# xulinfei1996/koordinator

Hardware: AMD Instinct MI355X
Metric: pods scheduled/sec + node-evals/sec (% HBM roofline) at 5k and 100k nodes (higher is better)
Workload: dtype int64; 1 GPU; C2: 10000 pods x 5000 nodes, NodeResourcesFit(LeastAllocated cpu/mem/batch-cpu/batch-mem) + LoadAwareScheduling(defaults) + ElasticQuota(32 leaf quotas); nodes=5000, percentage_of_nodes_to_score=100, parallelism=single-gpu, batch_pods=64, candidates=32

## Files before the change

koordinator_amd/csrc/koordgpu.hip:

```cpp
#include <hip/hip_runtime.h>

#include <algorithm>
#include <chrono>
#include <cmath>
#include <condition_variable>
#include <cstdio>
#include <cstdlib>
#include <cstring>
#include <mutex>
#include <string>
#include <unordered_map>
#include <unordered_set>
#include <vector>

#include <rccl/rccl.h>

#include "ks_pass.h"
#include "ks_mono.h"
#include "ks_plan.h"
#include "ks_fq.h"
#include "ks_debug.h"
#include "ks_topo.h"
#include "ks_preempt.h"
#include "ks_summary.h"
// ... 135 lines not shown
  r.h_mem = (double)r.mem * 100.0;
  r.gpu_core = s.gpu_core[i];
  r.gpu_mem = s.gpu_mem[i];
  r.gpu_ratio = s.gpu_ratio[i];
  if (r.gpu_core != 0 || r.gpu_mem != 0 || r.gpu_ratio != 0) r.flags |= kPodHasGpu | kPodGpuReq;
  r.rdma = s.rdma ? s.rdma[i] : 0;
  r.joint = s.joint ? s.joint[i] : 0u;
  r._pad0 = 0;
  if (r.rdma > 0) r.flags |= kPodHasGpu;
  if (dev_on && (r.flags & kPodHasGpu)) r.flags |= kPodDevNoNom;
  if ((r.flags & kPodHasGpu) || s.stat_dyn[i]) r.flags |= kPodNormDyn;
  if (s.topo && (s.topo[i].flags & KS_TOPO_DYN)) r.flags |= kPodTopoDyn;
  r.cpu_bind = (r.flags & KS_POD_CPU_BIND) ? ((s.cpu_bind[i] & 0x1Fu) | ((uint32_t)(r.cpu / 1000) << 8)) : 0u;
  out[i] = r;
}


struct SelectArgs {
  const uint2* __restrict__ in;
  const int32_t* __restrict__ cursor;
  uint32_t* cand_chunk;
  uint2* cand_t;
  uint64_t* cand_bound;
  uint64_t* cand_top;
  uint64_t* cand_second;
  int32_t* cand_count;
  int32_t* cand_total;
  int64_t nchunks;
  int64_t c0, c1;
  int32_t total_pods, batch, k;
  int32_t* next_base;
  const int32_t* real_cursor;
  const PodRec* pods;
};


constexpr int kSelHistBins = 1024;
constexpr int kSelThreads = 256;
constexpr int kSelUnroll = 8;
constexpr size_t kSelScratch = 128;
constexpr int kSelBlocks = 2 * kMaxBatch;
__host__ __device__ inline size_t select_smem(int64_t nc) { return (size_t)nc * sizeof(uint2) + kSelHistBins * 4 + kSelScratch; }

__global__ __launch_bounds__(kSelThreads) void select_kernel(SelectArgs a) {
  extern __shared__ __attribute__((aligned(16))) uint2 srow[];
  const int tid = threadIdx.x;
  const int lane = tid & 63;
  const int wv = tid >> 6;
  const int32_t cursor = __builtin_amdgcn_readfirstlane(*a.cursor);
  if (a.next_base && blockIdx.x == 0 && tid == 0) {
    const int32_t rc = *a.real_cursor;
    *a.next_base = (cursor == rc && cursor < a.total_pods) ? cursor + min(a.batch, a.total_pods - cursor) : rc;
  }
  if (cursor < a.total_pods && (__builtin_amdgcn_readfirstlane(a.pods[cursor].flags) & kPodTopoDyn)) return;
  if (cursor >= a.total_pods) return;
  const int32_t np = min(a.batch, a.total_pods - cursor);
  static_assert(kMaxBatch == 64, "the XCD mapping below: 4 XCDs x 16 pods (and ks_fq.h's per-pod records)");
  const int32_t xcd = (int32_t)(blockIdx.x & 7u);
  if (xcd >= kMaxBatch / 16) return;
  const int32_t p = xcd * 16 + (int32_t)(blockIdx.x >> 3);
  if (p >= np) return;
  const int32_t K = a.k;
  const int64_t nc = a.c1 - a.c0;
  const uint2* in = a.in + (size_t)a.c0 * kMaxBatch + p;
  uint32_t* hist = reinterpret_cast<uint32_t*>(srow + nc);
  uint64_t* xw = reinterpret_cast<uint64_t*>(hist + kSelHistBins);
  int32_t cnt = 0;
  uint32_t hmax = 0;
  uint64_t top = 0;
  for (int i = tid; i < kSelHistBins; i += kSelThreads) hist[i] = 0u;
  for (int64_t e0 = tid; e0 < nc; e0 += (int64_t)kSelThreads * kSelUnroll) {
    uint2 v[kSelUnroll];
#pragma unroll
    for (int u = 0; u < kSelUnroll; ++u) {
      const int64_t e = e0 + (int64_t)u * kSelThreads;
      v[u] = e < nc ? in[(size_t)e * kMaxBatch] : make_uint2(0u, 0u);
    }
#pragma unroll
    for (int u = 0; u < kSelUnroll; ++u) {
      const int64_t e = e0 + (int64_t)u * kSelThreads;
      if (e < nc) {
        srow[e] = v[u];
        const uint32_t h = v[u].x >> 6;
        cnt += h != 0;
        hmax = h > hmax ? h : hmax;
        top = umax64(top, local_gkey(v[u].x, a.c0 + e));
      }
    }
  }
  cnt = wave_sum_i32(cnt);
  hmax = wave_max_u32(hmax);
  top = wave_max_u64(top);
  if (lane == 0) {
    xw[wv] = top;
    xw[4 + wv] = (uint64_t)(uint32_t)cnt | ((uint64_t)hmax << 32);
  }
  __syncthreads();
  cnt = 0;
  hmax = 0;
  top = 0;
#pragma unroll
  for (int w = 0; w < kSelThreads / 64; ++w) {
    top = umax64(top, xw[w]);
    cnt += (int32_t)(uint32_t)xw[4 + w];
    const uint32_t hm = (uint32_t)(xw[4 + w] >> 32);
    hmax = hm > hmax ? hm : hmax;
  }
  uint32_t t = 1;
  int32_t need_eq = 0x7fffffff;
  const bool exhaustive = cnt <= K;
  const bool use_hist = !exhaustive && hmax < kSelHistBins;
  if (use_hist) {
    for (int64_t e = tid; e < nc; e += kSelThreads) {
      const uint32_t h = srow[e].x >> 6;
      if (h) atomicAdd(&hist[h], 1u);
    }
    __syncthreads();
  }
  if (wv != 0) return;
  if (!exhaustive) {
    if (use_hist) {
      constexpr int B = kSelHistBins / 64;
      uint32_t mine[B];
      uint32_t part = 0;
#pragma unroll
      for (int i = 0; i < B; ++i) {
        mine[i] = hist[lane * B + i];
        part += mine[i];
      }
      uint32_t suf = part;
#pragma unroll
      for (int off = 1; off < 64; off <<= 1) {
        const uint32_t v = __shfl_down(suf, off, 64);
        suf += (lane + off < 64) ? v : 0u;
      }
      const uint32_t suf_next = suf - part;
      const bool here = suf >= (uint32_t)K && suf_next < (uint32_t)K;
      uint32_t tl = 0, gtl = 0;
      if (here) {
        uint32_t acc = suf_next;
        for (int i = B - 1; i >= 0; --i) {
          if (acc + mine[i] >= (uint32_t)K) {
            tl = (uint32_t)(lane * B + i);
            gtl = acc;
            break;
          }
          acc += mine[i];
        }
      }
      const uint64_t hb = __ballot(here);
// ... 21 lines not shown
  uint64_t bound = 0, second = 0;
  const int64_t etop = top ? gkey_node(top) / 64 - a.c0 : -1;
  const uint64_t lanemask_lt = (lane == 0) ? 0ull : ((~0ull) >> (64 - lane));
  for (int64_t e0 = 0; e0 < nc; e0 += 64) {
    const int64_t e = e0 + lane;
    const uint2 loc = e < nc ? srow[e] : make_uint2(0u, 0u);
    second = umax64(second, local_gkey(e == etop ? loc.y : loc.x, a.c0 + e));
    const uint32_t h = loc.x >> 6;
    const bool is_gt = h > t;
    const bool is_eq = (h == t) && h != 0;
    const uint64_t beq = __ballot(is_eq);
    const int32_t eq_rank = eq_taken + __popcll(beq & lanemask_lt);
    const bool take_eq = is_eq && eq_rank < need_eq;
    const bool take = is_gt || take_eq;
    const uint64_t btake = __ballot(take);
    if (take) {
      const int32_t pos = base + __popcll(btake & lanemask_lt);
      a.cand_chunk[p * K + pos] = (uint32_t)(a.c0 + e);
      a.cand_t[p * K + pos] = loc;
      if (take_eq && eq_rank == need_eq - 1) bound = local_gkey(loc.x, a.c0 + e);
    }
    base += __popcll(btake);
    eq_taken += __popcll(beq);
  }
  bound = wave_max_u64(bound);
  second = wave_max_u64(second);
  if (lane == 0) {
    a.cand_count[p] = base;
    a.cand_total[p] = cnt;
    a.cand_bound[p] = exhaustive ? 0ull : bound;
    a.cand_top[p] = top;
    a.cand_second[p] = second;
  }
}



struct MergeArgs {
  const unsigned char* __restrict__ gather;
  const int32_t* __restrict__ cursor;
  uint32_t* cand_chunk;
  uint2* cand_t;
  uint64_t* cand_bound;
  uint64_t* cand_top;
  uint64_t* cand_second;
  int32_t* cand_count;
  int32_t nslots, total_pods, batch, k;
};

__global__ __launch_bounds__(64) void merge_kernel(MergeArgs a) {
  const int lane = threadIdx.x;
  const int32_t cursor = __builtin_amdgcn_readfirstlane(*a.cursor);
  if (cursor >= a.total_pods) return;
  const int32_t np = min(a.batch, a.total_pods - cursor);
  const int32_t p = blockIdx.x;
  if (p >= np) return;
  const int32_t K = a.k;
  const CandSlot L = cand_slot_layout(K);
  int32_t total = 0;
  uint64_t top = 0;
  for (int32_t s = 0; s < a.nslots; ++s) {
    const unsigned char* b = a.gather + (size_t)s * L.bytes;
    total += reinterpret_cast<const int32_t*>(b + L.total)[p];
    top = umax64(top, reinterpret_cast<const uint64_t*>(b + L.top)[p]);
  }
  auto entry = [&](int32_t s, int32_t i, uint32_t& chunk, uint2& t) {
// ... 732 lines not shown
  DevPtr<> evbuf;
  size_t evbuf_bytes = 0;
  DevPtr<> sumbuf;
  size_t sumbuf_bytes = 0;
  HostPtr sumhost;
  size_t sumhost_bytes = 0;
  DevPtr<> ures;
  DevPtr<> dscratch;
  size_t dscratch_bytes = 0;
  DevPtr<int2> cpuset_list;
  int32_t* cpuset_n = nullptr;
  CpuSet* cpuset_out = nullptr;
  uint32_t* cpuset_split = nullptr;
  int64_t* numa_alloc = nullptr;
  int32_t cpuset_cap = 0;
  DevPtr<uint32_t> cand_chunk;
  DevPtr<uint2> cand_t;
  DevPtr<uint64_t> cand_bound;
  DevPtr<uint64_t> cand_top;
  DevPtr<uint64_t> cand_second;
  DevPtr<> pre_rsv;
  DevPtr<int32_t> cand_total;
  DevPtr<int32_t> cand_count;
  DevPtr<int32_t> cursor;
  DevPtr<unsigned long long> counters;
  DevPtr<unsigned long long> dev_M;
  DevPtr<unsigned long long> dcache;
  int64_t dcache_words = 0;
  int32_t batch = 64, k = 32;
  int32_t k_cfg = 32;
  CommitPlan plan;
  bool commit_fq = true;
  bool fq_keys = true;
  int32_t nranks = 1, rank = 0, vshards = 1;
  ncclComm_t comm = nullptr;
  struct LoopGroup* loop = nullptr;
  hipEvent_t lev[2][2] = {};
  int64_t loop_seq = 0;
  DevPtr<unsigned long long> loop_scratch;
  DevPtr<unsigned char> gather;
  size_t gather_bytes = 0;
  hipStream_t sstream = nullptr;
  hipStream_t cstream = nullptr;
  DevPtr<int32_t> pipe;
  DevPtr<unsigned long long> pipe_top;
  int64_t pipe_k = 0;
  int32_t pipe_mode = -1;
  std::vector<Snap> snaps() const {
    std::vector<Snap> v;
    auto add = [&v](bool loaded, const auto& regions) {
      if (loaded) v.insert(v.end(), std::begin(regions), std::end(regions));
    };
    add(quota.blob.get(), quota.snap);
    add(dev.blob.get(), dev.snap);
    add(cpus.loaded, cpus.snap);
    add(numa.blob.get(), numa.snap);
    add(rsv.blob.get(), rsv.snap);
    return v;
  }
  ks_stats stats{};
};

#define KS_FAIL(ctx, code, ...)                                        \
  do {                                                                 \
    char buf_[512];                                                    \
    snprintf(buf_, sizeof(buf_), __VA_ARGS__);                         \
// ... 205 lines not shown
      return KS_EINVAL;
    }
  }
  if (cfg->reservation.enable) {
    const int64_t fitla = 100 * ((cfg->fit.enable_score ? cfg->fit.plugin_weight : 0) +
                                 (cfg->loadaware.enable_score ? cfg->loadaware.plugin_weight : 0) +
                                 (cfg->numa.enable ? cfg->numa.plugin_weight : 0) +
                                 (cfg->deviceshare.enable ? cfg->deviceshare.plugin_weight : 0) +
                                 (cfg->balanced.enable ? cfg->balanced.plugin_weight : 0) +
                                 (cfg->taint.enable_score ? cfg->taint.plugin_weight : 0) +
                                 (cfg->affinity.enable_score ? cfg->affinity.plugin_weight : 0));
    if (cfg->reservation.plugin_weight <= fitla || cfg->reservation.plugin_weight > ((int64_t)1 << 40) ||
        (fitla + 1) * (kRsvOrderBase + 1) >= (1 << 26)) {
      g_create_error = "ks_create: Reservation plugin weight must exceed 100 x (Fit + LoadAware weights) (ks_rsv.h ranking)";
      return KS_EUNSUPPORTED;
    }
  }
  int ndev = 0;
  if (hipGetDeviceCount(&ndev) != hipSuccess || ndev == 0) {
    g_create_error = "ks_create: no HIP device available";
    return KS_EHIP;
  }
  if (cfg->device < 0 || cfg->device >= ndev) {
    g_create_error = "ks_create: device ordinal out of range";
    return KS_EINVAL;
  }
  ks_ctx* ctx = new ks_ctx();
  ctx->cfg = *cfg;
  ctx->device = cfg->device;
  ctx->batch = cfg->batch_pods > 0 ? std::min(cfg->batch_pods, kMaxBatch) : 64;
  ctx->k = ctx->k_cfg = cfg->candidates > 0 ? std::min(cfg->candidates, kMaxCand) : 32;
  ctx->commit_fq = env_i64("KS_COMMIT_FQ", 1, 0, 1) != 0;
  ctx->fq_keys = env_i64("KS_FQ_KEYS", 1, 0, 1) != 0;
  if (hipSetDevice(ctx->device) != hipSuccess || hipStreamCreateWithFlags(&ctx->stream.h, hipStreamNonBlocking) != hipSuccess) {
    g_create_error = "ks_create: cannot create HIP stream";
    delete ctx;
    return KS_EHIP;
  }
  const size_t cand_bytes = (size_t)2 * kMaxBatch * kMaxCand;
  if (dev_alloc(ctx, ctx->cand_chunk, cand_bytes * 4) != KS_OK || dev_alloc(ctx, ctx->cand_t, cand_bytes * 8) != KS_OK ||
      dev_alloc(ctx, ctx->cand_bound, 2 * kMaxBatch * 8) != KS_OK || dev_alloc(ctx, ctx->cand_top, 2 * kMaxBatch * 8) != KS_OK ||
      dev_alloc(ctx, ctx->cand_second, 2 * kMaxBatch * 8) != KS_OK ||
      dev_alloc(ctx, ctx->pre_rsv, (size_t)kMaxBatch * kPreRsvM * sizeof(PreRsvT<kNumaWide>)) != KS_OK ||
      dev_alloc(ctx, ctx->cand_total, 2 * kMaxBatch * 4) != KS_OK || dev_alloc(ctx, ctx->cand_count, 2 * kMaxBatch * 4) != KS_OK ||
      dev_alloc(ctx, ctx->cursor, 64) != KS_OK || dev_alloc(ctx, ctx->counters, 256) != KS_OK ||
      dev_alloc(ctx, ctx->dev_M, kNormRows * kMaxBatch * 8) != KS_OK) {
    g_create_error = ctx->err;
    ks_destroy(ctx);
    return KS_ENOMEM;
  }
  if (hipMemsetAsync(ctx->cand_count.get(), list_fill(), 2 * kMaxBatch * 4, ctx->stream) != hipSuccess ||
      hipMemsetAsync(ctx->cand_chunk.get(), list_fill(), cand_bytes * 4, ctx->stream) != hipSuccess ||
      hipMemsetAsync(ctx->cand_t.get(), list_fill(), cand_bytes * 8, ctx->stream) != hipSuccess ||
      hipStreamSynchronize(ctx->stream) != hipSuccess) {
    g_create_error = "ks_create: cannot clear the candidate lists";
    ks_destroy(ctx);
    return KS_EHIP;
  }
  *out = ctx;
  return KS_OK;
}

void ks_destroy(ks_ctx* ctx) {
  if (!ctx) return;
  if (ctx->stream) (void)hipStreamSynchronize(ctx->stream);
  for (int i = 0; i < kPipeEvents; ++i) {
// ... 1715 lines not shown
      for (int t = 0; t < KS_AFFINITY_TERMS; ++t) {
        r.req[t] = pc->affinity_required[t] ? pc->affinity_required[t][i] : 0;
        r.pref[t] = pc->affinity_preferred[t] ? pc->affinity_preferred[t][i] : 0;
        r.w[t] = pc->affinity_weight[t] ? pc->affinity_weight[t][i] : 0;
        dyn |= (ctx->kc.aff & 2) && r.w[t] != 0;
      }
      r.pwant = pc->host_ports ? pc->host_ports[i] : 0;
      r.pconf = pc->host_ports_conflict ? pc->host_ports_conflict[i] : 0;
      hd[(size_t)i] = dyn ? 1 : 0;
    }
    if (p > 0) {
      HIPCHK(ctx, hipMemcpyAsync(st.stat, hs.data(), (size_t)p * sizeof(PodStat), hipMemcpyHostToDevice, ctx->stream));
      HIPCHK(ctx, hipMemcpyAsync(s.stat_dyn, hd.data(), (size_t)p, hipMemcpyHostToDevice, ctx->stream));
    }
    if (p > 0) {
      HIPCHK(ctx, hipStreamSynchronize(ctx->stream));
    }
  } else {
    HIPCHK(ctx, hipMemsetAsync(s.stat_dyn, 0, (size_t)p, ctx->stream));
  }
  return KS_OK;
}

static int prep_stage(ks_ctx* ctx, PodStage& st, int32_t p) {
  if (p <= 0) return KS_OK;
  const int threads = 256;
  hipLaunchKernelGGL(prep_pods_kernel, dim3((p + threads - 1) / threads), dim3(threads), 0, ctx->stream, st.cols,
                     st.recs, p, ctx->cfg.loadaware.scaling_cpu, ctx->cfg.loadaware.scaling_memory,
                     (int32_t)(ctx->cfg.deviceshare.enable != 0));
  HIPCHK(ctx, hipGetLastError());
  return KS_OK;
}

static int validate_pods(ks_ctx* ctx, const ks_pod_cols* pc, int32_t p) {
  if (ctx->cfg.topology.enable) {
    if ((pc->topo_term_beg == nullptr) != (pc->topo_terms == nullptr) || (pc->topo_prop_beg == nullptr) != (pc->topo_props == nullptr))
      KS_FAIL(ctx, KS_EINVAL, "topology lists: an offset array without its list (or the reverse)");
    for (int32_t i = 0; pc->topo_term_beg && i < p; ++i) {
      const int32_t b = pc->topo_term_beg[i], e = pc->topo_term_beg[i + 1];
      if ((i == 0 && b != 0) || e < b || e - b > KS_TOPO_MAX_TERMS)
        KS_FAIL(ctx, KS_EINVAL, "pod %d: topology term offsets [%d, %d) (at most %d terms)", i, b, e, KS_TOPO_MAX_TERMS);
      for (int32_t t = b; t < e; ++t) {
        const uint64_t w = pc->topo_terms[t];
        const int kind = (int)(w & 0xF), key = (int)((w >> 8) & 0xFF), prop = (int)((w >> 16) & 0xFFFF);
        const int32_t param = (int32_t)(uint32_t)(w >> 32);
        if (kind < KS_TOPO_K_SPREAD_HARD || kind > KS_TOPO_K_SCORE || prop >= ctx->topo.nprops || key > ctx->topo.nkeys ||
            ((w >> 5) & 0x7) != 0 ||
            ((kind == KS_TOPO_K_SPREAD_HARD || kind == KS_TOPO_K_SPREAD_SOFT) && param < 1) ||
            (kind == KS_TOPO_K_SCORE && (param < -1000000 || param > 1000000)))
          KS_FAIL(ctx, KS_EINVAL, "pod %d: topology term %d (%#llx) malformed", i, t - b, (unsigned long long)w);
      }
    }
    for (int32_t i = 0; pc->topo_prop_beg && i < p; ++i) {
      const int32_t b = pc->topo_prop_beg[i], e = pc->topo_prop_beg[i + 1];
      if ((i == 0 && b != 0) || e < b) KS_FAIL(ctx, KS_EINVAL, "pod %d: topology property offsets [%d, %d)", i, b, e);
      for (int32_t k = b; k < e; ++k)
        if (pc->topo_props[k] < 0 || pc->topo_props[k] >= ctx->topo.nprops)
          KS_FAIL(ctx, KS_EINVAL, "pod %d: topology property %d outside [0, %d)", i, pc->topo_props[k], ctx->topo.nprops);
    }
  }
  for (int32_t i = 0; pc->flags && i < p; ++i)
    if (pc->flags[i] & KS_POD_UNMODELLED)
      KS_FAIL(ctx, KS_EUNSUPPORTED, "pod %d: requests the library does not model (FPGA, DeviceShare allocate hints, "
                                    "a reserve pod as the scheduling subject)", i);
  for (int32_t i = 0; pc->affinity_required_n && i < p; ++i)
    if (pc->affinity_required_n[i] < 0 || pc->affinity_required_n[i] > KS_AFFINITY_TERMS)
// ... 168 lines not shown
  ca.n = ctx->nodes.n;
  ca.nchunks = ctx->nodes.nchunks;
  ca.total_pods = total;
  ca.batch = batch;
  ca.k = ctx->k;
  ca.rowcols = ctx->rowcols.get();
  ca.rcap = plan.rcap;
  ca.rsv_bytes = (int32_t)plan.rsv_bytes;
  ca.dev_bytes = (int32_t)plan.dev_bytes;
  ca.stat_lds = plan.stat_lds ? 1 : 0;
  ca.dv = ctx->ddv.get();
  ca.dev_M = ctx->dev_M.get();
  ca.cpuset_list = ctx->cpuset_list.get();
  ca.cpuset_n = ctx->cpuset_n;
  ca.cpuset_split = ctx->cpuset_split;
  ca.numa_alloc = ctx->numa_alloc;
  ca.force = 0;
  ca.numa_bytes = (int32_t)plan.numa_bytes;
  ca.nv = ctx->dnv.get();
  ca.pipe_base = nullptr;
  ca.carry = nullptr;
  ca.pipe_follow = nullptr;
  ca.pipe_after = nullptr;
  ca.top_reset = nullptr;
  ca.pre_rsv = nullptr;
  ca.topo = ctx->cfg.topology.enable && st.topo.get() ? 1 : 0;
  ca.topo_const = (int32_t)(100 * ctx->cfg.topology.spread_weight);
  ca.topo_rec = st.topo.get();
  ca.topo_props = st.topo_props.get();
  ca.topo_count = ctx->topo.count;
  ca.topo_npad = ctx->nodes.npad;
  ca.topo_best = ctx->topo.scr ? &ctx->topo.scr->best_total : nullptr;
  ca.nomq = nullptr;
  return ca;
}

static FqLaunch fq_launcher(int nsc) { return nsc == 0 ? fq_launch_n0() : (nsc == 2 ? fq_launch_n2() : fq_launch_n4()); }

static int commit_attr_set(ks_ctx* ctx) {
  static const int64_t env_general = env_i64("KS_COMMIT_GENERAL", 0, 0, 2);
  static const int64_t env_pre = env_i64("KS_PRE_RSV", 1, 0, 1);
  CommitPlanIn in{};
  in.kc = ctx->kc;
  in.k_cfg = ctx->k_cfg;
  in.nchunks = ctx->nodes.nchunks;
  in.nsc = ctx->nodes.nsc;
  in.numa_w = ctx->numa.w;
  in.q = ctx->quota.q.q;
  in.dev_held_any = ctx->rsv.dev_held_any;
  in.commit_fq = ctx->commit_fq;
  in.fq_keys = ctx->fq_keys;
  in.general_mode = (int)env_general;
  in.pre_rsv = env_pre != 0;
  const CommitPlan& plan = ctx->plan = commit_plan(in);
  if (plan.status == PlanStatus::kHeldWide)
    KS_FAIL(ctx, KS_EUNSUPPORTED,
            "reservations holding devices together with a NUMA-policy node with more than %d NUMA nodes", kNumaDev);
  ctx->k = plan.k;
  if (plan.status == PlanStatus::kTooLarge)
    KS_FAIL(ctx, KS_EUNSUPPORTED, "too many nodes for the commit kernel's LDS (%lld nodes, %zu B)", (long long)ctx->nodes.n, plan.smem);
  hipError_t e = pass_launcher(plan.feat, ctx->nodes.nsc, plan.wide).commit_attr(plan.qcache, plan.smem);
  if (e != hipSuccess) KS_FAIL(ctx, KS_EHIP, "hipFuncSetAttribute(commit LDS %zu): %s", plan.smem, hipGetErrorString(e));
  if (plan.fq) {
    e = fq_launcher(ctx->nodes.nsc).commit_attr(plan.fq_keys, plan.fq_smem);
    if (e != hipSuccess) KS_FAIL(ctx, KS_EHIP, "hipFuncSetAttribute(fq commit LDS %zu): %s", plan.fq_smem, hipGetErrorString(e));
  }
// ... 508 lines not shown
    } else if (k > 0) {
      HIPCHK(ctx, hipStreamWaitEvent(fs, ctx->pev_com[(k - 1) % kPipeEvents], 0));
    }
    sa.fix = carry;
    sa.fix_cursor = ctx->cursor.get();
    sa.ppw = pipe->fix_ppw;
    rec(3, fs);
    if (patch) {
      sa.list_t = cset.t;
      sa.list_chunk = cset.chunk;
      sa.list_count = cset.count;
      sa.list_bound = cset.bound;
      sa.list_top = ctx->pipe_top.get() + (size_t)(k & 1) * kMaxBatch;
      sa.list_k = ctx->k;
      le = pl.sweep(pipe->list_blocks, fs, sa);
    } else {
      sweep(pipe->fix_blocks, fs);
    }
    HIPCHK(ctx, le);
    rec(3, fs);
    return KS_OK;
  };
  if (pipe && !patch)
    if (int rc = fix(); rc != KS_OK) return rc;
  SelectArgs se;
  se.in = sout;
  se.cursor = base;
  se.nchunks = ctx->nodes.nchunks;
  se.total_pods = ctx->staged.np;
  se.batch = ctx->batch;
  se.k = ctx->k;
  se.real_cursor = ctx->cursor.get();
  se.pods = ctx->st.recs;
  const CandSlot L = cand_slot_layout(ctx->k);
  rec(1, ss);
  for (int32_t v = 0; v < ctx->vshards; ++v) {
    const int32_t sh = ctx->rank * ctx->vshards + v;
    se.c0 = shard_lo(sh);
    se.c1 = shard_lo(sh + 1);
    se.next_base = (pipe && !patch && v == 0) ? ctx->pipe.get() + ((k + 1) & 1) : nullptr;
    if (S == 1) {
      se.cand_chunk = cset.chunk;
      se.cand_t = cset.t;
      se.cand_bound = cset.bound;
      se.cand_top = cset.top;
      se.cand_second = cset.second;
      se.cand_count = cset.count;
      se.cand_total = cset.total;
    } else {
      unsigned char* b = ctx->gather.get() + (size_t)sh * L.bytes;
      se.cand_chunk = (uint32_t*)(b + L.chunk);
      se.cand_t = (uint2*)(b + L.t);
      se.cand_bound = cset.bound;
      se.cand_top = (uint64_t*)(b + L.top);
      se.cand_second = cset.second;
      se.cand_count = (int32_t*)(b + L.count);
      se.cand_total = (int32_t*)(b + L.total);
    }
    hipLaunchKernelGGL(select_kernel, dim3(kSelBlocks), dim3(kSelThreads), select_smem(se.c1 - se.c0), ss, se);
  }
  if (S > 1) {
    if (ctx->comm || ctx->loop)
      if (int rc = exchange_allgather(ctx, (size_t)ctx->vshards * L.bytes, ss); rc != KS_OK) return rc;
    MergeArgs ma;
    ma.gather = ctx->gather.get();
    ma.cursor = base;
// ... 18 lines not shown
    HIPCHK(ctx, hipEventRecord(ctx->pev_sel[k % kPipeEvents], ss));
    HIPCHK(ctx, hipStreamWaitEvent(cs, ctx->pev_sel[k % kPipeEvents], 0));
  }
  const CommitPlan& plan = ctx->plan;
  CommitArgs ca = commit_args(ctx, ctx->st, ctx->staged.np, ctx->batch);
  if (pipe) {
    ca.pipe_base = base;
    ca.carry = carry;
  }
  ca.cand_chunk = cset.chunk;
  ca.cand_t = cset.t;
  ca.cand_bound = cset.bound;
  ca.cand_top = cset.top;
  ca.cand_second = cset.second;
  ca.cand_count = cset.count;
  if (patch) {
    ca.pipe_follow = ctx->pipe.get() + ((k + 1) & 1);
    ca.pipe_after = base;
    ca.cand_top = (const uint64_t*)(ctx->pipe_top.get() + (size_t)(k & 1) * kMaxBatch);
    ca.top_reset = ctx->pipe_top.get() + (size_t)(k & 1) * kMaxBatch;
  }
  if (!plan.mono && !pipe && pl.reserve_pre && plan.pre_reserve) ca.pre_rsv = ctx->pre_rsv.get();
  rec(2, cs);
  if (ca.pre_rsv) HIPCHK(ctx, pl.reserve_pre(ctx->batch, cs, ca));
  if (ctx->nom.q_on) {
    ca.nomq = ctx->nom.dq;
    HIPCHK(ctx, pl.commit_nom(plan.qcache, plan.smem, cs, ca));
    if (ctx->nom.q_owners > 0) {
      hipLaunchKernelGGL((nom_retire_kernel<>), dim3(1), dim3(64), 0, cs, ctx->nom.q, (const ks_result*)ctx->st.results,
                         (const int32_t*)ctx->cursor.get(), ctx->counters.get());
      HIPCHK(ctx, hipGetLastError());
    }
  } else if (plan.mono) HIPCHK(ctx, pl.commit_mono(plan.qcache, plan.mono_smem, cs, ca));
  else if (plan.fq && !patch) HIPCHK(ctx, fq_launcher(ctx->nodes.nsc).commit(plan.fq_keys, plan.fq_smem, cs, ca));
  else HIPCHK(ctx, pl.commit(plan.qcache, plan.smem, cs, ca));
  rec(2, cs);
  if (pipe) HIPCHK(ctx, hipEventRecord(ctx->pev_com[k % kPipeEvents], cs));
  ctx->pipe_k = k + 1;
  return cores_pass_refresh(ctx);
}

static int schedule_staged_impl(ks_ctx* ctx) {
  if (!ctx->nodes.blob.get()) KS_FAIL(ctx, KS_ESTATE, "schedule before ks_load_nodes");
  if (!ctx->nom.q_staged) KS_NOM_REFUSE(ctx, "ks_schedule_staged");
  if (ctx->staged.stale)
    KS_FAIL(ctx, KS_ESTATE, "ks_schedule_staged: the staged batch predates a table reload; call ks_stage_pods again");
  ctx->nom.q_on = false;
  if (ctx->nom.q_staged && !ctx->nom.h_rows.empty()) {
    if (ctx->nranks * ctx->vshards > 1 || ctx->comm || ctx->loop)
      KS_FAIL(ctx, KS_EUNSUPPORTED, "ks_schedule_staged: a nominated table is loaded (%zu pods) and the nodes are sharded "
                                    "(ks_shard_init): the queue with a table runs on one shard only",
              ctx->nom.h_rows.size());
    ctx->nom.q_on = true;
  }
  HIPCHK(ctx, hipSetDevice(ctx->device));
  bind_mode(ctx, ctx->staged.bind_required);
  ctx->staged.cpusets_clobbered = false;
  ctx->stats = ks_stats{};
  const int32_t np = ctx->staged.np;
  if (np == 0) return KS_OK;
  {
    if (int rc = commit_attr_set(ctx); rc != KS_OK) return rc;
    hipError_t e = hipSuccess;
    if (ctx->nom.q_on) {
      const PassLaunch npl = pass_launcher(ctx->plan.feat, ctx->nodes.nsc, ctx->plan.wide);
      if (!npl.commit_nom || ctx->cfg.topology.enable)
        KS_FAIL(ctx, KS_EUNSUPPORTED, "ks_schedule_staged: a nominated table with a plugin set it is not modelled with");
// ... 31 lines not shown
  if (ppw > ctx->batch) ppw = ctx->batch;
  const int64_t nwork = std::max<int64_t>(local_chunks, 1) * ((ctx->batch + ppw - 1) / ppw);
  const int sweep_blocks = (int)((std::max<int64_t>(1, std::min<int64_t>((nwork + 3) / 4, env_cap)) + 7) & ~7ll);
  if (ensure_cpuset_bufs(ctx, np) != KS_OK) return KS_ENOMEM;
  hipEvent_t t0 = take_event(ctx, 0), t1 = take_event(ctx, 1);
  if (ctx->cpuset_list.get()) {
    HIPCHK(ctx, hipMemsetAsync(ctx->cpuset_n, 0, 4, ctx->stream));
    HIPCHK(ctx, hipMemsetAsync(ctx->cpuset_out, 0, (size_t)np * sizeof(CpuSet), ctx->stream));
    HIPCHK(ctx, hipMemsetAsync(ctx->numa_alloc, 0, (size_t)np * 2 * ctx->numa.w * 8, ctx->stream));
  }
  HIPCHK(ctx, hipMemsetAsync(ctx->cursor.get(), 0, 4, ctx->stream));
  HIPCHK(ctx, hipMemsetAsync(ctx->counters.get(), 0, 256, ctx->stream));
  PipeShape pshape{};
  const PipeShape* pipe = nullptr;
  if (!ctx->nom.q_on && pipelined(ctx)) {
    if (ensure_pipe(ctx) != KS_OK) return KS_EHIP;
    static const int64_t env_patch = env_i64("KS_PIPE_PATCH", 1, 0, 1);
    pshape.patch = env_patch != 0 && ctx->kc.monotone;
    static const int64_t env_fix_ppw = env_i64("KS_PIPE_FIX_PPW", 0, 1, kMaxBatch);
    pshape.fix_ppw = (int32_t)std::min<int64_t>(env_fix_ppw > 0 ? env_fix_ppw : (pshape.patch ? 16 : 2), ctx->batch);
    const int64_t fwork = (int64_t)kMaxBatch * ((ctx->batch + pshape.fix_ppw - 1) / pshape.fix_ppw);
    pshape.fix_blocks = (int)((std::max<int64_t>(1, (fwork + 3) / 4) + 7) & ~7ll);
    pshape.list_blocks = (int)((((int64_t)ctx->batch * ctx->k + 3) / 4 + 7) & ~7ll);
    pipe = &pshape;
    HIPCHK(ctx, hipMemsetAsync(ctx->pipe.get(), 0, kPipeWords * 4, ctx->stream));
    if (pshape.patch) {
      HIPCHK(ctx, hipMemsetD32Async((hipDeviceptr_t)(ctx->pipe.get() + 1), std::min(ctx->batch, np), 1, ctx->stream));
      HIPCHK(ctx, hipMemsetAsync(ctx->pipe_top.get(), 0, 2 * kMaxBatch * 8, ctx->stream));
    }
    ctx->pipe_k = 0;
  }
  HIPCHK(ctx, hipEventRecord(t0, ctx->stream));
  if (prep_stage(ctx, ctx->st, np) != KS_OK) return KS_EHIP;
  hipStream_t cs = pipe ? ctx->cstream : ctx->stream;
  if (pipe) {
    HIPCHK(ctx, hipEventRecord(ctx->pev_com[kPipeEvents - 1], ctx->stream));
    HIPCHK(ctx, hipStreamWaitEvent(ctx->sstream, ctx->pev_com[kPipeEvents - 1], 0));
    if (cs != ctx->stream) HIPCHK(ctx, hipStreamWaitEvent(cs, ctx->pev_com[kPipeEvents - 1], 0));
  }
  std::vector<std::pair<int, size_t>> evs;
  size_t evn = 2;
  int32_t host_cursor = 0;
  int rounds = 0;
  auto one_pass = [&](std::vector<std::pair<int, size_t>>* ev) -> int {
    switch (ctx->nodes.nsc) {
      case 0: return launch_pass<0>(ctx, ppw, sweep_blocks, pipe, ev, &evn);
      case 2: return launch_pass<2>(ctx, ppw, sweep_blocks, pipe, ev, &evn);
      default: return launch_pass<4>(ctx, ppw, sweep_blocks, pipe, ev, &evn);
    }
  };
  hipGraphExec_t gexec = nullptr;
  static const int64_t env_graph = env_i64("KS_TOPO_GRAPH", 1, 0, 1);
  constexpr int32_t kGraphIters = 4;
  if (ctx->cfg.topology.enable && ctx->st.ndyn > 0 && !pipe && !ctx->cfg.profile && env_graph && !ctx->comm && !ctx->loop) {
    EvBuf eb;
    if (ev_buffers(ctx, eb) != KS_OK) return KS_ENOMEM;
    hipGraph_t graph = nullptr;
    HIPCHK(ctx, hipStreamBeginCapture(ctx->stream, hipStreamCaptureModeThreadLocal));
    int rc = KS_OK;
    for (int32_t i = 0; i < kGraphIters && rc == KS_OK; ++i) rc = one_pass(nullptr);
    const hipError_t ee = hipStreamEndCapture(ctx->stream, &graph);
    if (rc != KS_OK) {
      if (graph) (void)hipGraphDestroy(graph);
      return rc;
    }
    HIPCHK(ctx, ee);
// ... 1236 lines not shown
```

koordinator_amd/csrc/ks_fq.h:

```cpp
#pragma once

#include "ks_pass.h"

namespace ks {

struct __attribute__((aligned(16))) FqPod {
  uint32_t qmeta;
  uint32_t flags;
  uint32_t qword;
  int32_t second;
  uint64_t bound, top;
};
static_assert(sizeof(FqPod) == 32, "FqPod layout");
static_assert(kMaxBatch == 64 && kMaxCand <= 64 && kQuotaLdsRows < 0xFFFF && KS_QUOTA_DIMS <= 8, "FqPod packing");

template <int NSC>
__device__ __forceinline__ uint64_t fq_rescan(const DevNodes* dnp, const Cfg& cfg, const PodRec& pod, int64_t chunk,
                                              uint64_t touched_mask, int64_t n) {
  const int lane = threadIdx.x & 63;
  const int64_t node = chunk * 64 + lane;
  asm volatile("" : "+s"(dnp));
  const DevNodes d = *dnp;
  NodeReg<NSC> r;
  load_node<NSC>(cfg, d, node, node < n, r);
  const EvalOut o = eval_pod_node<NSC, false>(cfg, pod, r);
  const bool skip = o.reasons || ((touched_mask >> lane) & 1ull);
  return wave_max_u64(skip ? 0ull : gkey(o.total, node));
}

template <int NSC, bool KEYS>
__global__ __launch_bounds__(commit_threads(0)) void commit_fq_kernel(CommitArgs a) {
  constexpr int NT = commit_threads(0);
  extern __shared__ __attribute__((aligned(16))) unsigned char smem_raw[];
  const int32_t K = a.k;
  const CommitLayout lay = commit_layout(K, a.nchunks, true, (size_t)a.rsv_bytes, (size_t)a.dev_bytes, (size_t)a.numa_bytes,
                                         a.q.q, true, false, KEYS);
  SlotRow* rows = reinterpret_cast<SlotRow*>(smem_raw + lay.rows);
  PodRec* spods = reinterpret_cast<PodRec*>(smem_raw + lay.pods);
  ks_result* sres = reinterpret_cast<ks_result*>(smem_raw + lay.res);
  int64_t* raw = reinterpret_cast<int64_t*>(smem_raw + lay.raw);
  int64_t* rawtop = reinterpret_cast<int64_t*>(smem_raw + lay.rawtop);
  int64_t* rawrun = reinterpret_cast<int64_t*>(smem_raw + lay.rawrun);
  int64_t* pqreq = reinterpret_cast<int64_t*>(smem_raw + lay.pqreq);
  uint2* cand_t = reinterpret_cast<uint2*>(smem_raw + lay.cand_t);
  uint32_t* cand_chunk = reinterpret_cast<uint32_t*>(smem_raw + lay.cand_chunk);
  FqPod* precs = reinterpret_cast<FqPod*>(smem_raw + lay.snuma);
  QuotaRowsLds qview = quota_lds(smem_raw + lay.quota, a.q.q);
  QuotaRowsLds* qlds = &qview;
  unsigned long long* touched = reinterpret_cast<unsigned long long*>(smem_raw + lay.touched);
  int2* hdesc = reinterpret_cast<int2*>(smem_raw + lay.help);
  int32_t* hpend = reinterpret_cast<int32_t*>(smem_raw + lay.help + (size_t)kMaxBatch * 8);
  int32_t* hdone = hpend + 1;
  int32_t* heval = hpend + 2;
  uint32_t* skey = reinterpret_cast<uint32_t*>(smem_raw + lay.skey);
  unsigned long long* hready = reinterpret_cast<unsigned long long*>(smem_raw + lay.help + (size_t)kMaxBatch * 8 + 16);
  const int tid = threadIdx.x;
  const int lane = tid & 63;
  const int32_t cursor0 = __builtin_amdgcn_readfirstlane(*a.cursor);
  if (cursor0 >= a.total_pods) {
    if (threadIdx.x == 0) pipe_next(a, cursor0);
    return;
  }
  if (pipe_bubble(a, cursor0)) return;
  const int32_t np = topo_pass_pods(a, cursor0, min(a.batch, a.total_pods - cursor0));
  if (np == 0) return;
#ifdef KS_COMMIT_STAMPS
  uint64_t ph[8] = {0, 0, 0, 0, 0, 0, 0, 0};
  uint64_t tlast = __builtin_amdgcn_s_memtime();
#define KS_FSTAMP(i)                                   \
  do {                                                 \
    const uint64_t t_ = __builtin_amdgcn_s_memtime(); \
    ph[i] += t_ - tlast;                               \
    tlast = t_;                                        \
  } while (0)
#else
#define KS_FSTAMP(i) \
  do {               \
  } while (0)
#endif

  lds_copy<NT>(cand_chunk, a.cand_chunk, np * K, tid);
  lds_copy<NT>(cand_t, a.cand_t, np * K, tid);
  for (int32_t i = tid; i < np * KS_QUOTA_DIMS; i += NT) {
    const int32_t p = i / KS_QUOTA_DIMS, dd = i - p * KS_QUOTA_DIMS;
    pqreq[i] = a.pq.req[dd][cursor0 + p];
  }
  {
    const int64_t* src = reinterpret_cast<const int64_t*>(a.pods + cursor0);
    int64_t* dst = reinterpret_cast<int64_t*>(spods);
    const int32_t words = np * (int32_t)(sizeof(PodRec) / 8);
    lds_copy<NT>(dst, src, words, tid);
  }
  for (int64_t c = tid; c < a.nchunks; c += NT) touched[c] = 0ull;
  lds_rawtop<NT>(rawtop, a.cand_top, a.rowcols, np, tid);
  lds_rawtop<NT>(rawrun, a.cand_second, a.rowcols, np, tid);
  for (int32_t r = tid; r < a.q.q; r += NT) {
    qlds->parent[r] = a.q.parent[r];
    qlds->limit_mask[r] = a.q.limit_mask[r];
    qlds->min_mask[r] = a.q.min_mask[r];
  }
  for (int32_t i = tid; i < a.q.q * KS_QUOTA_DIMS; i += NT) {
    qlds->limit[i] = a.q.limit[i];
    qlds->used[i] = a.q.used[i];
    qlds->min[i] = a.q.min[i];
    qlds->npused[i] = a.q.npused[i];
  }
  if (tid < 64 && lane < np) {
    const int32_t cnt = a.cand_count[lane];
    const uint64_t second = a.cand_second[lane];
    const uint32_t pmask = a.pq.mask[cursor0 + lane];
    const int32_t quota = a.pods[cursor0 + lane].quota;
    FqPod r;
    r.bound = a.cand_bound[lane];
    r.top = a.cand_top[lane];
    r.flags = a.pods[cursor0 + lane].flags;
    r.qmeta = 0xFFFFu;
    if (quota >= 0) {
      const int32_t pp = a.q.parent[quota];
      r.qmeta = (uint32_t)(pp < 0 ? 0xFFFF : pp) | ((a.q.limit_mask[quota] & 0xFFu) << 16) |
                ((a.q.min_mask[quota] & 0xFFu) << 24);
    }
    r.qword = (uint32_t)(quota < 0 ? 0xFFFF : quota) | ((pmask & 0xFFu) << 16) | ((uint32_t)max(0, min(cnt, 64)) << 24);
    r.second = (int32_t)gkey_node(second);
    precs[lane] = r;
  }
  const void* my_col = nullptr;
  int32_t my_w = 8;
  if (tid < RF_N) {
    my_col = a.rowcols[lane].p;
    my_w = a.rowcols[lane].width;
  }
  if (tid == 0) {
    *hpend = 0;
    *hdone = 0;
    heval[0] = 0;
    heval[1] = 0;
    *hready = 0ull;
  }
  __syncthreads();
  if (tid >= (KEYS ? 192 : 128)) return;
  KS_FSTAMP(0);
  Cfg cfg{};
  {
    auto pin = [](int32_t v) {
      asm volatile("" : "+s"(v));
      return v;
    };
    cfg.fit_filter = pin(a.c.fit_filter);
    cfg.fit_score = pin(a.c.fit_score);
    cfg.fw_cpu = pin(a.c.fw_cpu);
    cfg.fw_mem = pin(a.c.fw_mem);
    cfg.fw_eph = pin(a.c.fw_eph);
#pragma unroll
    for (int k = 0; k < NSC; ++k) cfg.fw_sc[k] = pin(a.c.fw_sc[k]);
    cfg.fit_pw = pin(a.c.fit_pw);
    cfg.la_filter = pin(a.c.la_filter);
    cfg.la_score = pin(a.c.la_score);
    cfg.la_prod_usage = pin(a.c.la_prod_usage);
    cfg.lw_cpu = pin(a.c.lw_cpu);
    cfg.lw_mem = pin(a.c.lw_mem);
    cfg.la_pw = pin(a.c.la_pw);
    cfg.quota_enable = 1;
    cfg.quota_parent = pin(a.c.quota_parent);
// ... 307 lines not shown
  if (lane < nslots) {
    const DevNodes d = *a.dn;
    const SlotRow& r = rows[lane];
    const int64_t node = snode;
    gst(d.req_cpu + node, r.t[ST_FREE_CPU].c - r.t[ST_FREE_CPU].h);
    gst(d.req_mem + node, r.t[ST_FREE_MEM].c - r.t[ST_FREE_MEM].h);
    gst(d.req_eph + node, r.t[ST_FREE_EPH].c - r.t[ST_FREE_EPH].h);
    gst(d.nz_cpu + node, term_requested(r.t[ST_CPU]));
    gst(d.nz_mem + node, term_requested(r.t[ST_MEM]));
#pragma unroll
    for (int k = 0; k < KS_MAX_SCALARS; ++k) gst(d.req_sc[k] + node, r.t[ST_FREE_SC + k].c - r.t[ST_FREE_SC + k].h);
    gst(d.pod_count + node, r.pod_count);
    gst(d.la_term_cpu + node, term_requested(r.t[ST_LCPU]));
    gst(d.la_term_mem + node, term_requested(r.t[ST_LMEM]));
    gst(d.la_pterm_cpu + node, term_requested(r.t[ST_PLCPU]));
    gst(d.la_pterm_mem + node, term_requested(r.t[ST_PLMEM]));
  }
  for (int32_t i = lane; i < a.q.q * KS_QUOTA_DIMS; i += 64) {
    a.q.used[i] = qlds->used[i];
    a.q.npused[i] = qlds->npused[i];
  }
  pipe_carry(a, nslots, snode);
  if (a.top_reset) a.top_reset[lane] = 0ull;
  if (lane == 0) {
    *a.cursor = cursor0 + processed;
    pipe_next(a, cursor0 + processed);
    atomicAdd(&a.counters[0], 1ull);
    if (processed < np) atomicAdd(&a.counters[1], 1ull);
    atomicAdd(&a.counters[2], (unsigned long long)rescans);
    atomicAdd(&a.counters[3], (unsigned long long)misses);
    atomicAdd(&a.counters[15], (unsigned long long)fast);
#ifdef KS_COMMIT_STAMPS
    for (int i = 0; i < 7; ++i) atomicAdd(&a.counters[8 + i], (unsigned long long)ph[i]);
#endif
  }
#undef KS_FSTAMP
}

struct FqLaunch {
  hipError_t (*commit)(bool keys, size_t smem, hipStream_t s, const CommitArgs& a);
  hipError_t (*commit_attr)(bool keys, size_t smem);
};
FqLaunch fq_launch_n0();
FqLaunch fq_launch_n2();
FqLaunch fq_launch_n4();

}
```

koordinator_amd/csrc/ks_pass.h:

```cpp
#pragma once

#include <hip/hip_runtime.h>

#include <type_traits>

#include "ks_device.h"
#include "ks_rsv.h"
#include "ks_dev.h"
#include "ks_cpuset.h"
#include "ks_numa.h"
#include "ks_topo.h"
#include "ks_nominated.h"

namespace ks {

__device__ __forceinline__ uint64_t local_gkey(uint32_t loc, int64_t chunk) {
  if (loc == 0) return 0;
  const int64_t node = chunk * 64 + (63 - (int64_t)(loc & 63u));
  return ((uint64_t)(loc >> 6) << 32) | (uint64_t)(0xFFFFFFFFu - (uint32_t)node);
}


struct SweepArgs {
  const DevNodes* __restrict__ dn;
// ... 280 lines not shown
  const uint2* __restrict__ cand_t;
  const uint64_t* __restrict__ cand_bound;
  const uint64_t* __restrict__ cand_top;
  const uint64_t* __restrict__ cand_second;
  const int32_t* __restrict__ cand_count;
  ks_result* results;
  unsigned long long* counters;
  int64_t n, nchunks;
  int32_t total_pods, batch, k;
  int2* cpuset_list;
  int32_t* cpuset_n;
  uint32_t* cpuset_split;
  int64_t* numa_alloc;
  int32_t force;
  int32_t rcap;
  int32_t rsv_bytes;
  int32_t dev_bytes;
  int32_t numa_bytes;
  int32_t stat_lds;
  const int32_t* pipe_base;
  int32_t* carry;
  const int32_t* pipe_follow;
  int32_t* pipe_after;
  unsigned long long* top_reset;
  const void* pre_rsv;
  int32_t topo;
  int32_t topo_const;
  const TopoRec* topo_rec;
  const int32_t* topo_props;
  int32_t* topo_count;
  int64_t topo_npad;
  const long long* topo_best;
  const DevNomQueue* nomq;
};

template <bool NOM>
__device__ __forceinline__ int32_t nom_pass_pods(const CommitArgs& a, int32_t cursor0, int32_t np) {
  if constexpr (NOM) {
    const int lane = threadIdx.x & 63;
    const NomPod* wp = a.nomq->pods;
    const uint64_t own = __ballot(lane < np && gld(&wp[cursor0 + lane].owner) != 0);
    if (own) {
      const int32_t f = (int32_t)(__ffsll((long long)own) - 1);
      return f == 0 ? 1 : f;
    }
  }
  return np;
}

constexpr int kPreRsvM = 16;
template <int W>
struct __attribute__((aligned(16))) PreRsvT {
  int32_t node;
  uint32_t flags;
  uint32_t reasons, affinity;
  int64_t alloc[2][W];
  int32_t cpus[W];
  uint32_t gminors, rminors;
  int32_t _pad[2];
  int64_t g_core, g_mem, g_ratio, g_rdma;
};
using PreRsv = PreRsvT<kNumaDev>;
static_assert(sizeof(PreRsv) == 144 && sizeof(PreRsvT<kNumaWide>) == 224, "PreRsv layout");

__device__ __forceinline__ void pipe_next(const CommitArgs& a, int32_t rc) {
  if (!a.pipe_after) return;
// ... 1634 lines not shown
```

Measured before the change: 602,700 pods/s.

## Stage FQ commit prologue data in select kernel and batch-issue prologue loads

```diff
diff --git a/koordinator_amd/csrc/koordgpu.hip b/koordinator_amd/csrc/koordgpu.hip
--- a/koordinator_amd/csrc/koordgpu.hip
+++ b/koordinator_amd/csrc/koordgpu.hip
@@ -191,6 +191,9 @@
   int32_t* next_base;
   const int32_t* real_cursor;
   const PodRec* pods;
+  FqPassRec* fq_rec;
+  const uint2* fq_words;
+  const RowCol* rowcols;
 };
 
 
@@ -224,6 +227,16 @@
   const uint2* in = a.in + (size_t)a.c0 * kMaxBatch + p;
   uint32_t* hist = reinterpret_cast<uint32_t*>(srow + nc);
   uint64_t* xw = reinterpret_cast<uint64_t*>(hist + kSelHistBins);
+  RowCol rcol{nullptr, 8, 0};
+  uint2 fqw = make_uint2(0u, 0u);
+  uint32_t pflags = 0;
+  if (a.fq_rec && wv < 2) {
+    rcol = a.rowcols[lane & (RF_N - 1)];
+    if (wv == 0) {
+      fqw = a.fq_words[cursor + p];
+      pflags = a.pods[cursor + p].flags;
+    }
+  }
   int32_t cnt = 0;
   uint32_t hmax = 0;
   uint64_t top = 0;
@@ -275,6 +288,10 @@
       if (h) atomicAdd(&hist[h], 1u);
     }
     __syncthreads();
+  }
+  if (a.fq_rec && wv == 1 && lane < RF_N) {
+    const int64_t v = load_field(rcol.p, rcol.width, top ? gkey_node(top) : 0);
+    a.fq_rec[p].top[lane] = top ? v : 0;
   }
   if (wv != 0) return;
   if (!exhaustive) {
@@ -362,6 +379,29 @@
     a.cand_top[p] = top;
     a.cand_second[p] = second;
   }
+  if (a.fq_rec) {
+    FqPassRec* rec = a.fq_rec + p;
+    if (lane < RF_N) {
+      const int64_t v = load_field(rcol.p, rcol.width, second ? gkey_node(second) : 0);
+      rec->run[lane] = second ? v : 0;
+    }
+    if (lane == 0) {
+      FqPod r;
+      r.qmeta = fqw.x;
+      r.flags = pflags;
+      r.qword = fqw.y | ((uint32_t)max(0, min(base, 64)) << 24);
+      r.second = (int32_t)gkey_node(second);
+      r.bound = exhaustive ? 0ull : bound;
+      r.top = top;
+      rec->pod = r;
+    }
+  }
+}
+
+__global__ void prep_fq_words_kernel(const PodRec* pods, const uint32_t* pmask, DevQuotas q, uint2* out, int32_t np) {
+  const int32_t i = blockIdx.x * blockDim.x + threadIdx.x;
+  if (i >= np) return;
+  out[i] = fq_step_words(pods[i].quota, pmask[i], q);
 }
 
 
@@ -1160,6 +1200,11 @@
   CommitPlan plan;
   bool commit_fq = true;
   bool fq_keys = true;
+  bool fq_staged = true;
+  bool fq_run = false;
+  DevPtr<FqPassRec> fq_rec;
+  DevPtr<uint2> fq_words;
+  int32_t fq_words_cap = 0;
   int32_t nranks = 1, rank = 0, vshards = 1;
   ncclComm_t comm = nullptr;
   struct LoopGroup* loop = nullptr;
@@ -1431,6 +1476,7 @@
   ctx->k = ctx->k_cfg = cfg->candidates > 0 ? std::min(cfg->candidates, kMaxCand) : 32;
   ctx->commit_fq = env_i64("KS_COMMIT_FQ", 1, 0, 1) != 0;
   ctx->fq_keys = env_i64("KS_FQ_KEYS", 1, 0, 1) != 0;
+  ctx->fq_staged = env_i64("KS_FQ_STAGED", 1, 0, 1) != 0;
   if (hipSetDevice(ctx->device) != hipSuccess || hipStreamCreateWithFlags(&ctx->stream.h, hipStreamNonBlocking) != hipSuccess) {
     g_create_error = "ks_create: cannot create HIP stream";
     delete ctx;
@@ -3212,6 +3258,21 @@
   return KS_OK;
 }
 
+static int prep_fq_words(ks_ctx* ctx, PodStage& st, int32_t p) {
+  if (p <= 0) return KS_OK;
+  if (!ctx->fq_rec.get() && dev_alloc(ctx, ctx->fq_rec, (size_t)kMaxBatch * sizeof(FqPassRec)) != KS_OK) return KS_ENOMEM;
+  if (ctx->fq_words_cap < p) {
+    ctx->fq_words_cap = 0;
+    if (dev_alloc(ctx, ctx->fq_words, (size_t)p * sizeof(uint2)) != KS_OK) return KS_ENOMEM;
+    ctx->fq_words_cap = p;
+  }
+  const int threads = 256;
+  hipLaunchKernelGGL(prep_fq_words_kernel, dim3((p + threads - 1) / threads), dim3(threads), 0, ctx->stream,
+                     (const PodRec*)st.recs, (const uint32_t*)st.pq.mask, ctx->quota.q, ctx->fq_words.get(), p);
+  HIPCHK(ctx, hipGetLastError());
+  return KS_OK;
+}
+
 static int validate_pods(ks_ctx* ctx, const ks_pod_cols* pc, int32_t p) {
   if (ctx->cfg.topology.enable) {
     if ((pc->topo_term_beg == nullptr) != (pc->topo_terms == nullptr) || (pc->topo_prop_beg == nullptr) != (pc->topo_props == nullptr))
@@ -3446,6 +3507,7 @@
   ca.topo_npad = ctx->nodes.npad;
   ca.topo_best = ctx->topo.scr ? &ctx->topo.scr->best_total : nullptr;
   ca.nomq = nullptr;
+  ca.fq_rec = nullptr;
   return ca;
 }
 
@@ -4020,6 +4082,9 @@
   se.k = ctx->k;
   se.real_cursor = ctx->cursor.get();
   se.pods = ctx->st.recs;
+  se.fq_rec = ctx->fq_run ? ctx->fq_rec.get() : nullptr;
+  se.fq_words = ctx->fq_words.get();
+  se.rowcols = ctx->rowcols.get();
   const CandSlot L = cand_slot_layout(ctx->k);
   rec(1, ss);
   for (int32_t v = 0; v < ctx->vshards; ++v) {
@@ -4104,7 +4169,10 @@
       HIPCHK(ctx, hipGetLastError());
     }
   } else if (plan.mono) HIPCHK(ctx, pl.commit_mono(plan.qcache, plan.mono_smem, cs, ca));
-  else if (plan.fq && !patch) HIPCHK(ctx, fq_launcher(ctx->nodes.nsc).commit(plan.fq_keys, plan.fq_smem, cs, ca));
+  else if (plan.fq && !patch) {
+    ca.fq_rec = se.fq_rec;
+    HIPCHK(ctx, fq_launcher(ctx->nodes.nsc).commit(plan.fq_keys, plan.fq_smem, cs, ca));
+  }
   else HIPCHK(ctx, pl.commit(plan.qcache, plan.smem, cs, ca));
   rec(2, cs);
   if (pipe) HIPCHK(ctx, hipEventRecord(ctx->pev_com[k % kPipeEvents], cs));
@@ -4202,6 +4270,9 @@
   }
   HIPCHK(ctx, hipEventRecord(t0, ctx->stream));
   if (prep_stage(ctx, ctx->st, np) != KS_OK) return KS_EHIP;
+  ctx->fq_run = ctx->fq_staged && ctx->plan.fq && !ctx->plan.mono && !ctx->nom.q_on && S == 1 && !(pipe && pipe->patch);
+  if (ctx->fq_run)
+    if (int rc = prep_fq_words(ctx, ctx->st, np); rc != KS_OK) return rc;
   hipStream_t cs = pipe ? ctx->cstream : ctx->stream;
   if (pipe) {
     HIPCHK(ctx, hipEventRecord(ctx->pev_com[kPipeEvents - 1], ctx->stream));
diff --git a/koordinator_amd/csrc/ks_fq.h b/koordinator_amd/csrc/ks_fq.h
--- a/koordinator_amd/csrc/ks_fq.h
+++ b/koordinator_amd/csrc/ks_fq.h
@@ -13,6 +13,42 @@
 };
 static_assert(sizeof(FqPod) == 32, "FqPod layout");
 static_assert(kMaxBatch == 64 && kMaxCand <= 64 && kQuotaLdsRows < 0xFFFF && KS_QUOTA_DIMS <= 8, "FqPod packing");
+
+__device__ __forceinline__ uint2 fq_step_words(int32_t quota, uint32_t pmask, const DevQuotas& q) {
+  uint32_t qmeta = 0xFFFFu;
+  if (quota >= 0) {
+    const int32_t pp = q.parent[quota];
+    qmeta = (uint32_t)(pp < 0 ? 0xFFFF : pp) | ((q.limit_mask[quota] & 0xFFu) << 16) | ((q.min_mask[quota] & 0xFFu) << 24);
+  }
+  return make_uint2(qmeta, (uint32_t)(quota < 0 ? 0xFFFF : quota) | ((pmask & 0xFFu) << 16));
+}
+
+struct __attribute__((aligned(16))) FqPassRec {
+  FqPod pod;
+  int64_t top[32], run[32];
+};
+static_assert(sizeof(FqPassRec) == 544 && RF_N == 32, "FqPassRec layout");
+
+typedef uint32_t Quad __attribute__((ext_vector_type(4)));
+
+template <int N, int NT, typename T>
+struct ProCopy {
+  T v[N];
+  __device__ __forceinline__ void issue(const T* src, int32_t n, int tid) {
+#pragma unroll
+    for (int u = 0; u < N; ++u) {
+      const int32_t i = tid + u * NT;
+      v[u] = src[i < n ? i : 0];
+    }
+  }
+  __device__ __forceinline__ void store(T* dst, int32_t n, int tid) const {
+#pragma unroll
+    for (int u = 0; u < N; ++u) {
+      const int32_t i = tid + u * NT;
+      if (i < n) dst[i] = v[u];
+    }
+  }
+};
 
 template <int NSC>
 __device__ __forceinline__ uint64_t fq_rescan(const DevNodes* dnp, const Cfg& cfg, const PodRec& pod, int64_t chunk,
@@ -79,56 +115,122 @@
   } while (0)
 #endif
 
-  lds_copy<NT>(cand_chunk, a.cand_chunk, np * K, tid);
-  lds_copy<NT>(cand_t, a.cand_t, np * K, tid);
-  for (int32_t i = tid; i < np * KS_QUOTA_DIMS; i += NT) {
-    const int32_t p = i / KS_QUOTA_DIMS, dd = i - p * KS_QUOTA_DIMS;
-    pqreq[i] = a.pq.req[dd][cursor0 + p];
-  }
-  {
-    const int64_t* src = reinterpret_cast<const int64_t*>(a.pods + cursor0);
-    int64_t* dst = reinterpret_cast<int64_t*>(spods);
-    const int32_t words = np * (int32_t)(sizeof(PodRec) / 8);
-    lds_copy<NT>(dst, src, words, tid);
-  }
   for (int64_t c = tid; c < a.nchunks; c += NT) touched[c] = 0ull;
-  lds_rawtop<NT>(rawtop, a.cand_top, a.rowcols, np, tid);
-  lds_rawtop<NT>(rawrun, a.cand_second, a.rowcols, np, tid);
-  for (int32_t r = tid; r < a.q.q; r += NT) {
-    qlds->parent[r] = a.q.parent[r];
-    qlds->limit_mask[r] = a.q.limit_mask[r];
-    qlds->min_mask[r] = a.q.min_mask[r];
-  }
-  for (int32_t i = tid; i < a.q.q * KS_QUOTA_DIMS; i += NT) {
-    qlds->limit[i] = a.q.limit[i];
-    qlds->used[i] = a.q.used[i];
-    qlds->min[i] = a.q.min[i];
-    qlds->npused[i] = a.q.npused[i];
-  }
-  if (tid < 64 && lane < np) {
-    const int32_t cnt = a.cand_count[lane];
-    const uint64_t second = a.cand_second[lane];
-    const uint32_t pmask = a.pq.mask[cursor0 + lane];
-    const int32_t quota = a.pods[cursor0 + lane].quota;
-    FqPod r;
-    r.bound = a.cand_bound[lane];
-    r.top = a.cand_top[lane];
-    r.flags = a.pods[cursor0 + lane].flags;
-    r.qmeta = 0xFFFFu;
-    if (quota >= 0) {
-      const int32_t pp = a.q.parent[quota];
-      r.qmeta = (uint32_t)(pp < 0 ? 0xFFFF : pp) | ((a.q.limit_mask[quota] & 0xFFu) << 16) |
-                ((a.q.min_mask[quota] & 0xFFu) << 24);
-    }
-    r.qword = (uint32_t)(quota < 0 ? 0xFFFF : quota) | ((pmask & 0xFFu) << 16) | ((uint32_t)max(0, min(cnt, 64)) << 24);
-    r.second = (int32_t)gkey_node(second);
-    precs[lane] = r;
-  }
   const void* my_col = nullptr;
   int32_t my_w = 8;
   if (tid < RF_N) {
     my_col = a.rowcols[lane].p;
     my_w = a.rowcols[lane].width;
+  }
+  if (a.fq_rec) {
+    constexpr int kRecW = (int)(sizeof(FqPassRec) / 16), kPodW = (int)(sizeof(PodRec) / 16);
+    constexpr int kNL = (kMaxBatch * kMaxCand + NT - 1) / NT, kNQ = (kQuotaLdsRows * KS_QUOTA_DIMS + NT - 1) / NT;
+    constexpr int kNR = (kQuotaLdsRows + NT - 1) / NT, kNP = (kMaxBatch * KS_QUOTA_DIMS + NT - 1) / NT;
+    ProCopy<kNL, NT, uint32_t> c_chunk;
+    ProCopy<kNL, NT, uint2> c_t;
+    ProCopy<(kMaxBatch * kPodW + NT - 1) / NT, NT, Quad> c_pods;
+    ProCopy<(kMaxBatch * kRecW + NT - 1) / NT, NT, Quad> c_rec;
+    ProCopy<kNR, NT, int32_t> c_par;
+    ProCopy<kNR, NT, uint32_t> c_lm, c_mm;
+    ProCopy<kNQ, NT, int64_t> c_lim, c_used, c_min, c_npu;
+    const int32_t nl = np * K, nq = a.q.q, nqd = nq * KS_QUOTA_DIMS, nrec = np * kRecW, npq = np * KS_QUOTA_DIMS;
+    c_rec.issue(reinterpret_cast<const Quad*>(a.fq_rec), nrec, tid);
+    c_chunk.issue(a.cand_chunk, nl, tid);
+    c_t.issue(a.cand_t, nl, tid);
+    c_pods.issue(reinterpret_cast<const Quad*>(a.pods + cursor0), np * kPodW, tid);
+    int64_t rq[kNP];
+    const int64_t* qcol[KS_QUOTA_DIMS];
+#pragma unroll
+    for (int d = 0; d < KS_QUOTA_DIMS; ++d) {
+      qcol[d] = a.pq.req[d];
+      asm volatile("" : "+s"(qcol[d]));
+    }
+#pragma unroll
+    for (int u = 0; u < kNP; ++u) {
+      const int32_t i = tid + u * NT, ii = i < npq ? i : 0;
+      const int32_t p = ii / KS_QUOTA_DIMS, dd = ii - p * KS_QUOTA_DIMS;
+      const int64_t* col = qcol[0];
+#pragma unroll
+      for (int d = 1; d < KS_QUOTA_DIMS; ++d) col = dd == d ? qcol[d] : col;
+      rq[u] = gld(col + cursor0 + p);
+    }
+    c_par.issue(a.q.parent, nq, tid);
+    c_lm.issue(a.q.limit_mask, nq, tid);
+    c_mm.issue(a.q.min_mask, nq, tid);
+    c_lim.issue(a.q.limit, nqd, tid);
+    c_used.issue(a.q.used, nqd, tid);
+    c_min.issue(a.q.min, nqd, tid);
+    c_npu.issue(a.q.npused, nqd, tid);
+    asm volatile("" ::: "memory");
+#pragma unroll
+    for (int u = 0; u < (kMaxBatch * kRecW + NT - 1) / NT; ++u) {
+      const int32_t i = tid + u * NT;
+      if (i < nrec) {
+        const int32_t p = i / kRecW, w = i - p * kRecW;
+        Quad* dst = w < 2    ? reinterpret_cast<Quad*>(precs) + p * 2 + w
+                     : w < 18 ? reinterpret_cast<Quad*>(rawtop) + p * 16 + (w - 2)
+                              : reinterpret_cast<Quad*>(rawrun) + p * 16 + (w - 18);
+        *dst = c_rec.v[u];
+      }
+    }
+    c_chunk.store(cand_chunk, nl, tid);
+    c_t.store(cand_t, nl, tid);
+    c_pods.store(reinterpret_cast<Quad*>(spods), np * kPodW, tid);
+#pragma unroll
+    for (int u = 0; u < kNP; ++u)
+      if (tid + u * NT < npq) pqreq[tid + u * NT] = rq[u];
+    c_par.store(qlds->parent, nq, tid);
+    c_lm.store(qlds->limit_mask, nq, tid);
+    c_mm.store(qlds->min_mask, nq, tid);
+    c_lim.store(qlds->limit, nqd, tid);
+    c_used.store(qlds->used, nqd, tid);
+    c_min.store(qlds->min, nqd, tid);
+    c_npu.store(qlds->npused, nqd, tid);
+  } else {
+    lds_copy<NT>(cand_chunk, a.cand_chunk, np * K, tid);
+    lds_copy<NT>(cand_t, a.cand_t, np * K, tid);
+    for (int32_t i = tid; i < np * KS_QUOTA_DIMS; i += NT) {
+      const int32_t p = i / KS_QUOTA_DIMS, dd = i - p * KS_QUOTA_DIMS;
+      pqreq[i] = a.pq.req[dd][cursor0 + p];
+    }
+    {
+      const int64_t* src = reinterpret_cast<const int64_t*>(a.pods + cursor0);
+      int64_t* dst = reinterpret_cast<int64_t*>(spods);
+      const int32_t words = np * (int32_t)(sizeof(PodRec) / 8);
+      lds_copy<NT>(dst, src, words, tid);
+    }
+    lds_rawtop<NT>(rawtop, a.cand_top, a.rowcols, np, tid);
+    lds_rawtop<NT>(rawrun, a.cand_second, a.rowcols, np, tid);
+    for (int32_t r = tid; r < a.q.q; r += NT) {
+      qlds->parent[r] = a.q.parent[r];
+      qlds->limit_mask[r] = a.q.limit_mask[r];
+      qlds->min_mask[r] = a.q.min_mask[r];
+    }
+    for (int32_t i = tid; i < a.q.q * KS_QUOTA_DIMS; i += NT) {
+      qlds->limit[i] = a.q.limit[i];
+      qlds->used[i] = a.q.used[i];
+      qlds->min[i] = a.q.min[i];
+      qlds->npused[i] = a.q.npused[i];
+    }
+    if (tid < 64 && lane < np) {
+      const int32_t cnt = a.cand_count[lane];
+      const uint64_t second = a.cand_second[lane];
+      const uint32_t pmask = a.pq.mask[cursor0 + lane];
+      const int32_t quota = a.pods[cursor0 + lane].quota;
+      FqPod r;
+      r.bound = a.cand_bound[lane];
+      r.top = a.cand_top[lane];
+      r.flags = a.pods[cursor0 + lane].flags;
+      r.qmeta = 0xFFFFu;
+      if (quota >= 0) {
+        const int32_t pp = a.q.parent[quota];
+        r.qmeta = (uint32_t)(pp < 0 ? 0xFFFF : pp) | ((a.q.limit_mask[quota] & 0xFFu) << 16) |
+                  ((a.q.min_mask[quota] & 0xFFu) << 24);
+      }
+      r.qword = (uint32_t)(quota < 0 ? 0xFFFF : quota) | ((pmask & 0xFFu) << 16) | ((uint32_t)max(0, min(cnt, 64)) << 24);
+      r.second = (int32_t)gkey_node(second);
+      precs[lane] = r;
+    }
   }
   if (tid == 0) {
     *hpend = 0;
@@ -502,6 +604,8 @@
     atomicAdd(&a.counters[15], (unsigned long long)fast);
 #ifdef KS_COMMIT_STAMPS
     for (int i = 0; i < 7; ++i) atomicAdd(&a.counters[8 + i], (unsigned long long)ph[i]);
+#else
+    if (a.fq_rec) atomicAdd(&a.counters[14], 1ull);
 #endif
   }
 #undef KS_FSTAMP
diff --git a/koordinator_amd/csrc/ks_pass.h b/koordinator_amd/csrc/ks_pass.h
--- a/koordinator_amd/csrc/ks_pass.h
+++ b/koordinator_amd/csrc/ks_pass.h
@@ -336,6 +336,7 @@
   int64_t topo_npad;
   const long long* topo_best;
   const DevNomQueue* nomq;
+  const void* fq_rec;
 };
 
 template <bool NOM>
```

New measurement: 633,000 pods/s, median of 6. 1.05x the previous value.
